# ningw42/GPU_Stereo_Matching

Measured on AMD Instinct MI355X. Metric: disparity-maps/sec + ms/frame, 1080p d_max=128, higher is better.
Workload: dtype u8; 1 GPU; cfg3: 1920x1080 synthetic rectified pairs, 11x11 SAD box aggregation + WTA (bit-exact with getDisp/kernalFindCorr), d_max=128; the path BASELINE.md's GPU-target table and the north star's >=100x CPU BlockMatching.cpp target are quoted on; BASELINE configs[2]'s guided-filter aggregation of the same frames: 'cfg3_guided'; width=1920, height=1080, num_disp=128, radius=5, seed=1234, parallelism=frame-parallel x1

## Files before the change

gpu_stereo_matching_amd/csrc/bm_box_mfma.hip:

```cpp
#include <atomic>
#include <type_traits>

#include "bm_common.h"

namespace sm {
namespace {

typedef _Float16 h2 __attribute__((ext_vector_type(2)));
typedef _Float16 h8 __attribute__((ext_vector_type(8)));
typedef float f4 __attribute__((ext_vector_type(4)));
typedef uint32_t u4 __attribute__((ext_vector_type(4)));

constexpr int kT = 64;
constexpr int kNW = 4;
constexpr int kThreads = 64 * kNW;
constexpr int kColB = 128;
constexpr uint32_t kInfBits = 0x7F800000u;

template <int R, int DMAX, int NP>
struct MG {
    static_assert(NP == 1 || NP == 2, "one or two disparities per pass");
    static constexpr int NOB = NP == 2 ? 3 : 4;
    static constexpr int NXB = (NP == 1 || R <= 6) ? 4 : 3;
    static constexpr int TOY = NOB == 4 ? kT - 2 * R : 16 * NOB;
    static constexpr int TOX = NXB == 4 ? kT - 2 * R : 16 * NXB;
    static constexpr int FOLD = 16 * NXB + 1;
    static constexpr int RC = kT + DMAX;
    static constexpr int RS_BYTES = RC * kColB;
    static constexpr int L_BYTES = kT * kColB;
    static constexpr int LDS_BYTES = L_BYTES + RS_BYTES;
    static constexpr int BIAS = ((2 * R + 1) * 255 + 1) / 2;
    static constexpr int KEEP = RC - TOX;
    static constexpr int NEW0 = KEEP & ~3;
    static constexpr int NEW4 = (RC - NEW0) / 4;
    static constexpr int MOVE_U = (KEEP * 8 + kThreads - 1) / kThreads;
    static_assert(TOY + 2 * R <= kT && TOX + 2 * R <= kT, "every output's window lies in the input tile");
    static_assert(8 * NEW4 + 8 * (kT / 4) <= kThreads, "a carried tile stages in one pass");
    static_assert(TOY * FOLD * 4 <= L_BYTES + TOX * kColB,
                  "the fold plane aliases the left tile and the band columns the next tile drops, none it keeps");
    static_assert(BIAS < 2048 && (2 * R + 1) * 255 - BIAS < 2048, "D1 exact in f16");
    static_assert((int64_t)(2 * R + 1) * (2 * R + 1) * 255 * 256 + 255 < (1 << 24), "keys exact in f32");
};

__device__ __forceinline__ int slot(int col, int q) { return col * kColB + ((q ^ ((col >> 1) & 7)) << 4); }

__device__ __forceinline__ uint32_t ld_u32(const uint8_t* p, int y, int x, int W, int H, int pitch) {
    if (y < 0 || y >= H) return 0u;
    const uint8_t* row = p + (int64_t)y * pitch;
    if (x >= 0 && x + 3 < W) {
        uint32_t v;
        __builtin_memcpy(&v, row + x, 4);
        return v;
    }
    uint32_t v = 0;
#pragma unroll
    for (int b = 0; b < 4; ++b)
        if (x + b >= 0 && x + b < W) v |= (uint32_t)row[x + b] << (8 * b);
    return v;
}

__device__ __forceinline__ void stage_pack(const uint32_t (&w)[8], uint8_t* dst, int col, int q) {
#pragma unroll
    for (int b = 0; b < 4; ++b) {
        u4 v;
#pragma unroll
        for (int m = 0; m < 4; ++m)
            v[m] = 0x64006400u | ((w[2 * m] >> (8 * b)) & 0xFFu) | (((w[2 * m + 1] >> (8 * b)) & 0xFFu) << 16);
        *reinterpret_cast<u4*>(dst + slot(col + b, q)) = v;
    }
}

template <int NC4>
__device__ __forceinline__ void stage_cols(const uint8_t* img, int ytop, int xleft, int W, int H, int pitch,
                                           uint8_t* dst, int tid) {
    for (int e = tid; e < 8 * NC4; e += kThreads) {
        const int q = e / NC4, j = e - q * NC4;
        uint32_t w[8];
#pragma unroll
        for (int i = 0; i < 8; ++i) w[i] = ld_u32(img, ytop + 8 * q + i, xleft + 4 * j, W, H, pitch);
        stage_pack(w, dst, 4 * j, q);
    }
}

template <int NEW0, int NEW4>
struct CarriedElem {
    bool right;
    int q, col, dx;
    __device__ __forceinline__ explicit CarriedElem(int tid) {
        constexpr int NR = 8 * NEW4, NL = 8 * (kT / 4);
        const int e = min(tid, NR + NL - 1);
        right = e < NR;
        const int el = e - NR;
        q = right ? e / NEW4 : el / (kT / 4);
        dx = 4 * (right ? e - q * NEW4 : el - q * (kT / 4));
        col = (right ? NEW0 : 0) + dx;
    }
};

__device__ __forceinline__ int per_tile(int tid) {
    asm volatile("" : "+v"(tid));
    return tid;
}

constexpr uint32_t kAbsBits = 0x7FFF7FFFu;

__device__ __forceinline__ u4 abs_diff(u4 l, u4 r, uint32_t keep) {
    u4 ad;
#pragma unroll
    for (int m = 0; m < 4; ++m) {
        const uint32_t lm = l[m], rm = r[m];
        const h2 d = __builtin_bit_cast(h2, lm) - __builtin_bit_cast(h2, rm);
        ad[m] = __builtin_bit_cast(uint32_t, d) & keep;
    }
    return ad;
}

__device__ __forceinline__ uint2 pack_f16(f4 v) {
    uint2 p;
    p.x = __builtin_bit_cast(uint32_t, __builtin_amdgcn_cvt_pkrtz(v[0], v[1]));
    p.y = __builtin_bit_cast(uint32_t, __builtin_amdgcn_cvt_pkrtz(v[2], v[3]));
    return p;
}

__device__ __forceinline__ f4 mfma(u4 a, u4 b, f4 c) {
    return __builtin_amdgcn_mfma_f32_16x16x32_f16(__builtin_bit_cast(h8, a), __builtin_bit_cast(h8, b), c, 0, 0, 0);
}

template <int R, int DMAX, int NP, bool WALK>
__device__ __forceinline__ void box_mfma_tiles(const MatchArgs& a, int tiles_x, int tiles_y, int per, int rem) {
    using G = MG<R, DMAX, NP>;
    constexpr int NXB = G::NXB, NOB = G::NOB;
    extern __shared__ __attribute__((aligned(16))) uint8_t smem[];
    uint8_t* lsm = smem;
    uint8_t* rsm = smem + G::L_BYTES;

    const int tid = threadIdx.x;
    const int wave = __builtin_amdgcn_readfirstlane(tid >> 6);
    const int lane = tid & 63;
    const int l16 = lane & 15;
    const int g = lane >> 4;

    const int wg = xcd_tile(blockIdx.x, gridDim.x);
    int t_begin = wg * per, t_end = t_begin + per;
    if (WALK && rem != 0) {
        t_begin += (int)((int64_t)wg * rem / (int)gridDim.x);
        t_end += (int)((int64_t)(wg + 1) * rem / (int)gridDim.x);
    }
    if constexpr (!WALK) t_end = t_begin + 1;
    if (t_begin >= t_end) return;
    const int tiles = tiles_x * tiles_y;
    int frame = t_begin / tiles;
    int ty = (t_begin - frame * tiles) / tiles_x;
    int tx = t_begin - frame * tiles - ty * tiles_x;
    const int W = a.W, H = a.H;
    const int d_lo = a.d_lo, d_hi = a.d_hi;

    u4 bv0, bvm, bvp;
    u4 bh, bhs;
#pragma unroll
    for (int m = 0; m < 4; ++m) {
        uint32_t w0 = 0, wm = 0, wp = 0, wh = 0, ws = 0;
#pragma unroll
        for (int e = 0; e < 2; ++e) {
            const int j = 2 * m + e;
            const int dv = 8 * g + j - l16;
            const int xin = j < 4 ? 4 * g + j : 16 + 4 * g + (j - 4);
            const int dh = xin - l16;
            const int ds = (j < 4 ? 16 + 4 * g + j : 4 * g + (j - 4)) - l16;
            w0 |= (dv >= 0 && dv <= 2 * R ? 0x3C00u : 0u) << (16 * e);
            wm |= (dv - 16 >= 0 && dv - 16 <= 2 * R ? 0x3C00u : 0u) << (16 * e);
            wp |= (dv + 16 >= 0 && dv + 16 <= 2 * R ? 0x3C00u : 0u) << (16 * e);
            wh |= (dh >= 0 && dh <= 2 * R ? 0x5C00u : 0u) << (16 * e);
            ws |= (ds >= 0 && ds <= 2 * R ? 0x5C00u : 0u) << (16 * e);
        }
        bv0[m] = w0;
        bvm[m] = wm;
        bvp[m] = wp;
        bh[m] = wh;
        bhs[m] = ws;
    }
    const float nbias = -(float)G::BIAS;
    const f4 c1 = {nbias, nbias, nbias, nbias};
    const float c2base = (float)(256 * (2 * R + 1) * G::BIAS);

    const int laddr = slot(l16, g);

    bool carried = false;
#pragma unroll 1
    for (int tile = t_begin;; ++tile) {
        const int x0 = tx * G::TOX;
        const int y0 = ty * G::TOY;
        const uint8_t* Lf = a.left + (int64_t)frame * a.frame_stride;
        const uint8_t* Rf = a.right + (int64_t)frame * a.frame_stride;

        if (!carried) {
            const int band0 = x0 - R - d_lo - DMAX;
            const int st = per_tile(tid);
            stage_cols<G::RC / 4>(Rf, y0 - R, band0, W, H, a.pitch, rsm, st);
            stage_cols<kT / 4>(Lf, y0 - R, x0 - R, W, H, a.pitch, lsm, st);
        }

        uint32_t best[NOB][NXB][4];
#pragma unroll
        for (int ob = 0; ob < NOB; ++ob)
#pragma unroll
            for (int xb = 0; xb < NXB; ++xb)
#pragma unroll
                for (int i = 0; i < 4; ++i) best[ob][xb][i] = kInfBits;

        const int d_end = min(d_hi, W - x0 + 1);
        const int nd = max(d_end - d_lo, 0);
        const int dw_lo = d_lo + (wave * nd) / kNW;
        const int dw_hi = d_lo + ((wave + 1) * nd) / kNW;
        const int d_free = W - (min(x0 + G::TOX, W) - 1);
        const int d_m = (x0 - R + kT > W) ? d_lo : max(min(x0 - R, d_free) + 1, d_lo);
        const int n_free = max(min(dw_hi, d_m) - dw_lo, 0);
        const int dw_m = dw_lo + n_free - n_free % NP;

        const bool carry_next = WALK && tile + 1 < t_end && tx + 1 < tiles_x;
        const int nxl = x0 + G::TOX - R, nxr = nxl - d_lo - DMAX + G::NEW0;
        const bool prefetch = carry_next && y0 - R >= 0 && y0 - R + kT <= H && nxr >= 0 && nxl + kT <= W;
        uint32_t pw[8];
        if (prefetch) {
            const CarriedElem<G::NEW0, G::NEW4> ce(per_tile(tid));
            const uint8_t* p = (ce.right ? Rf : Lf) + (int64_t)(y0 - R + 8 * ce.q) * a.pitch +
                               ((ce.right ? nxr : nxl) + ce.dx);
#pragma unroll
            for (int i = 0; i < 8; ++i) __builtin_memcpy(&pw[i], p + (int64_t)i * a.pitch, 4);
        }

        __syncthreads();

        auto run = [&](auto masked_c, const int lo, const int hi) {
            constexpr bool MASKED = decltype(masked_c)::value;
#pragma unroll 1
            for (int d = lo; d < hi; d += NP) {
                const int dd[2] = {d, min(d + 1, hi - 1)};
                int raddr[NP];
                float c2v[NP];
                f4 c2[NP];
#pragma unroll
                for (int p = 0; p < NP; ++p) {
                    raddr[p] = slot(l16 + DMAX + d_lo - dd[p], g);
                    c2v[p] = c2base + (float)dd[p];
                    c2[p] = f4{c2v[p], c2v[p], c2v[p], c2v[p]};
                }
                const int laddr_d = laddr + (int)((uint32_t)d >> 31);
                u4 t[NP][NOB];
#pragma unroll
                for (int cb = 0; cb <= NXB; ++cb) {
                    if (cb < 4) {
                        const u4 l0 = *reinterpret_cast<const u4*>(lsm + laddr_d + cb * 16 * kColB);
                        const u4 l1 = *reinterpret_cast<const u4*>(lsm + (laddr_d ^ 64) + cb * 16 * kColB);
#pragma unroll
                        for (int p = 0; p < NP; ++p) {
                            const u4 r0 = *reinterpret_cast<const u4*>(rsm + raddr[p] + cb * 16 * kColB);
                            const u4 r1 = *reinterpret_cast<const u4*>(rsm + (raddr[p] ^ 64) + cb * 16 * kColB);
                            uint32_t keep = kAbsBits;
                            if constexpr (MASKED) {
                                const int c0 = __builtin_amdgcn_readfirstlane(x0 - R + 16 * cb - dd[p]);
                                keep = (uint32_t)(l16 + c0) < (uint32_t)(W - dd[p]) ? kAbsBits : 0u;
                            }
                            const u4 ad0 = abs_diff(l0, r0, keep);
                            const u4 ad1 = abs_diff(l1, r1, keep);
                            f4 sv[4];
                            sv[0] = mfma(ad0, bv0, c1);
                            sv[1] = mfma(ad0, bvm, c1);
                            sv[1] = mfma(ad1, bvp, sv[1]);
                            sv[2] = mfma(ad1, bv0, c1);
                            if constexpr (NOB == 4) sv[3] = mfma(ad1, bvm, c1);
#pragma unroll
                            for (int ob = 0; ob < NOB; ++ob) {
                                const uint2 pk = pack_f16(sv[ob]);
                                t[p][ob][2 * (cb & 1)] = pk.x;
                                t[p][ob][2 * (cb & 1) + 1] = pk.y;
                            }
                        }
                    }
                    if constexpr (NP == 2) __builtin_amdgcn_sched_barrier(0);
                    if (cb >= 1) {
                        const int xb = cb - 1;
                        f4 c2x[NP];
#pragma unroll
                        for (int p = 0; p < NP; ++p) {
                            c2x[p] = c2[p];
                            if constexpr (MASKED) {
                                const int e = __builtin_amdgcn_readfirstlane(W - x0 - 16 * xb - dd[p]) - 4 * g;
#pragma unroll
                                for (int i = 0; i < 4; ++i)
                                    c2x[p][i] = i <= e ? c2v[p] : __builtin_bit_cast(float, kInfBits);
                            }
                        }
#pragma unroll
                        for (int ob = 0; ob < NOB; ++ob) {
                            u4 o[NP];
#pragma unroll
                            for (int p = 0; p < NP; ++p)
                                o[p] = __builtin_bit_cast(u4, mfma((cb & 1) ? bh : bhs, t[p][ob], c2x[p]));
#pragma unroll
                            for (int i = 0; i < 4; ++i) {
                                uint32_t k = o[0][i];
#pragma unroll
                                for (int p = 1; p < NP; ++p) k = min(k, o[p][i]);
                                best[ob][xb][i] = min(best[ob][xb][i], k);
                            }
                        }
                    }
                    if constexpr (NP == 2) __builtin_amdgcn_sched_barrier(0);
                }
            }
        };
        run(std::false_type{}, dw_lo, dw_m);
        run(std::true_type{}, dw_m, dw_hi);

        __syncthreads();

        uint32_t* fold = reinterpret_cast<uint32_t*>(smem);
        if (wave == 0) {
#pragma unroll
            for (int ob = 0; ob < NOB; ++ob)
#pragma unroll
                for (int xb = 0; xb < NXB; ++xb)
#pragma unroll
                    for (int i = 0; i < 4; ++i)
                        fold[(16 * ob + l16) * G::FOLD + 16 * xb + 4 * g + i] = best[ob][xb][i];
        }
        __syncthreads();
        if (wave != 0) {
#pragma unroll
            for (int ob = 0; ob < NOB; ++ob)
#pragma unroll
                for (int xb = 0; xb < NXB; ++xb)
#pragma unroll
                    for (int i = 0; i < 4; ++i)
                        atomicMin(&fold[(16 * ob + l16) * G::FOLD + 16 * xb + 4 * g + i], best[ob][xb][i]);
        }
        __syncthreads();
        uint8_t* Df = a.disp ? a.disp + (int64_t)frame * a.out_frame_stride : nullptr;
        uint32_t* Kf = a.keys ? a.keys + (int64_t)frame * W * H : nullptr;
        if (lane < G::TOX && x0 + lane < W) {
            const int ylim = min(G::TOY, H - y0);
            uint8_t* drow = Df ? Df + (int64_t)y0 * a.out_pitch + x0 + lane : nullptr;
            uint32_t* krow = Kf ? Kf + (int64_t)y0 * W + x0 + lane : nullptr;
            for (int j = wave; j < ylim; j += kNW) {
                const uint32_t kb = fold[j * G::FOLD + lane];
                const uint32_t kf = kb >= kInfBits ? 0xFFFFFFFFu : (uint32_t)__builtin_bit_cast(float, kb);
                const uint32_t k = min(kf, a.seed_key);
                if (drow) drow[(int64_t)j * a.out_pitch] = k < a.thresh_key ? (uint8_t)(k & 0xFFu) : (uint8_t)0;
                if (krow) krow[(int64_t)j * W] = k;
            }
        }

        if (tile + 1 == t_end) break;
        carried = carry_next;
        if (++tx == tiles_x) {
            tx = 0;
            if (++ty == tiles_y) {
                ty = 0;
                ++frame;
            }
        }
        if (!carried) {
            __syncthreads();
            continue;
        }
        const int mt = per_tile(tid);
        u4 mv[G::MOVE_U];
#pragma unroll
        for (int i = 0; i < G::MOVE_U; ++i) {
            const int u = min(mt + i * kThreads, G::KEEP * 8 - 1);
            mv[i] = *reinterpret_cast<const u4*>(rsm + slot((u >> 3) + G::TOX, u & 7));
        }
        __syncthreads();
#pragma unroll
        for (int i = 0; i < G::MOVE_U; ++i) {
            const int u = min(mt + i * kThreads, G::KEEP * 8 - 1);
            *reinterpret_cast<u4*>(rsm + slot(u >> 3, u & 7)) = mv[i];
        }
        const CarriedElem<G::NEW0, G::NEW4> ce(mt);
        if (!prefetch) {
#pragma unroll
            for (int i = 0; i < 8; ++i)
                pw[i] = ld_u32(ce.right ? Rf : Lf, y0 - R + 8 * ce.q + i, (ce.right ? nxr : nxl) + ce.dx, W, H,
                               a.pitch);
        }
        stage_pack(pw, ce.right ? rsm : lsm, ce.col, ce.q);
    }
}

template <int R, int DMAX, int NP>
__global__ __launch_bounds__(kThreads, 3) void box_mfma_kernel(MatchArgs a, int tiles_x, int tiles_y, int per,
                                                                int rem) {
    box_mfma_tiles<R, DMAX, NP, true>(a, tiles_x, tiles_y, per, rem);
}

template <int R, int DMAX>
__global__ __launch_bounds__(kThreads, 3) void box_mfma_tile_kernel(MatchArgs a, int tiles_x, int tiles_y) {
    box_mfma_tiles<R, DMAX, 1, false>(a, tiles_x, tiles_y, 1, 0);
}

constexpr int kMaxDevices = 64;
constexpr int kRangesPerSlot = 16;

template <int R, int DMAX, int NP>
hipError_t resident_workgroups(int* out) {
    static std::atomic<int> slots[kMaxDevices];
    int dev = 0;
    hipError_t e = hipGetDevice(&dev);
    if (e != hipSuccess) return e;
    const bool cached = dev >= 0 && dev < kMaxDevices;
    int v = cached ? slots[dev].load(std::memory_order_relaxed) : 0;
    if (v == 0) {
        int per_cu = 0, cus = 0;
        e = hipOccupancyMaxActiveBlocksPerMultiprocessor(&per_cu, box_mfma_kernel<R, DMAX, NP>, kThreads,
                                                         (size_t)MG<R, DMAX, NP>::LDS_BYTES);
        if (e != hipSuccess) return e;
        e = hipDeviceGetAttribute(&cus, hipDeviceAttributeMultiprocessorCount, dev);
        if (e != hipSuccess) return e;
        v = (per_cu > 0 ? per_cu : 1) * (cus > 0 ? cus : 1);
        if (cached) slots[dev].store(v, std::memory_order_relaxed);
    }
    *out = v;
    return hipSuccess;
}

template <int R, int DMAX, int NP>
hipError_t launch_rdp(const MatchArgs& a, int batch, hipStream_t s, int workgroups) {
    using G = MG<R, DMAX, NP>;
    const int tiles_x = (a.W + G::TOX - 1) / G::TOX;
    const int tiles_y = (a.H + G::TOY - 1) / G::TOY;
    const int64_t total = (int64_t)tiles_x * tiles_y * batch;
    if (total <= 0 || total > 0x7FFFFFFF || workgroups < 0) return hipErrorInvalidValue;
    int64_t n = workgroups;
    if constexpr (NP == 1) {
        if (n == 0 || n >= total) {
            hipLaunchKernelGGL((box_mfma_tile_kernel<R, DMAX>), dim3((unsigned)total), dim3(kThreads),
                               (size_t)G::LDS_BYTES, s, a, tiles_x, tiles_y);
            return hipGetLastError();
        }
    }
    if (n == 0) {
        int slots = 0;
        hipError_t e = resident_workgroups<R, DMAX, NP>(&slots);
        if (e != hipSuccess) return e;
        n = (int64_t)slots * kRangesPerSlot;
    }
    if (n > total) n = total;
    hipLaunchKernelGGL((box_mfma_kernel<R, DMAX, NP>), dim3((unsigned)n), dim3(kThreads), (size_t)G::LDS_BYTES, s, a,
                       tiles_x, tiles_y, (int)(total / n), (int)(total % n));
    return hipGetLastError();
}

template <int R, int DMAX>
hipError_t launch_rd(const MatchArgs& a, int batch, hipStream_t s, int workgroups) {
    if constexpr (DMAX == 64 && R <= 2) {
        if (a.d_hi - a.d_lo <= 32) return launch_rdp<R, DMAX, 1>(a, batch, s, workgroups);
    }
    return launch_rdp<R, DMAX, 2>(a, batch, s, workgroups);
}

template <int R>
hipError_t launch_r(const MatchArgs& a, int batch, hipStream_t s, int workgroups) {
    const int dspan = a.d_hi - a.d_lo;
    if (dspan <= 64) return launch_rd<R, 64>(a, batch, s, workgroups);
    if (dspan <= 128) return launch_rd<R, 128>(a, batch, s, workgroups);
    if (dspan <= 192) return launch_rd<R, 192>(a, batch, s, workgroups);
    return launch_rd<R, 256>(a, batch, s, workgroups);
}

}

bool box_mfma_scope(const MatchArgs& a) {
    return a.radius >= 1 && a.radius <= kMaxFastRadius && a.valid_mode == 0 && a.d_lo >= 0 && a.d_hi > a.d_lo &&
           a.d_hi <= kMaxDisp;
}

hipError_t launch_box_match_mfma(const MatchArgs& a, int batch, hipStream_t s, int workgroups) {
    if (!box_mfma_scope(a)) return hipErrorInvalidValue;
    switch (a.radius) {
        case 1: return launch_r<1>(a, batch, s, workgroups);
        case 2: return launch_r<2>(a, batch, s, workgroups);
        case 3: return launch_r<3>(a, batch, s, workgroups);
        case 4: return launch_r<4>(a, batch, s, workgroups);
        case 5: return launch_r<5>(a, batch, s, workgroups);
        case 6: return launch_r<6>(a, batch, s, workgroups);
        case 7: return launch_r<7>(a, batch, s, workgroups);
        default: return hipErrorInvalidValue;
    }
}

}
```

Before: 25990 disparity-maps/s.

## Hand-schedule paired-disparity MFMA loop and defer next-tile prefetch

Adds a dedicated unmasked loop for the two-disparities-per-pass path. It interleaves LDS fetches, f16 abs-diff, vertical and horizontal MFMA stages and min-reductions, with explicit sched_barrier slots so the next column block's loads and second-stage MFMAs overlap the first-stage work. For NP==2 the next-tile global prefetch is moved after the main loop instead of before it, which frees registers during the hot loop. The hand scheduling is rigid and may raise register pressure or serialise badly if the compiler's choices were already good.

```diff
diff --git a/gpu_stereo_matching_amd/csrc/bm_box_mfma.hip b/gpu_stereo_matching_amd/csrc/bm_box_mfma.hip
--- a/gpu_stereo_matching_amd/csrc/bm_box_mfma.hip
+++ b/gpu_stereo_matching_amd/csrc/bm_box_mfma.hip
@@ -221,13 +221,16 @@
         const int nxl = x0 + G::TOX - R, nxr = nxl - d_lo - DMAX + G::NEW0;
         const bool prefetch = carry_next && y0 - R >= 0 && y0 - R + kT <= H && nxr >= 0 && nxl + kT <= W;
         uint32_t pw[8];
-        if (prefetch) {
-            const CarriedElem<G::NEW0, G::NEW4> ce(per_tile(tid));
-            const uint8_t* p = (ce.right ? Rf : Lf) + (int64_t)(y0 - R + 8 * ce.q) * a.pitch +
-                               ((ce.right ? nxr : nxl) + ce.dx);
-#pragma unroll
-            for (int i = 0; i < 8; ++i) __builtin_memcpy(&pw[i], p + (int64_t)i * a.pitch, 4);
-        }
+        auto issue_prefetch = [&] {
+            if (prefetch) {
+                const CarriedElem<G::NEW0, G::NEW4> ce(per_tile(tid));
+                const uint8_t* p = (ce.right ? Rf : Lf) + (int64_t)(y0 - R + 8 * ce.q) * a.pitch +
+                                   ((ce.right ? nxr : nxl) + ce.dx);
+#pragma unroll
+                for (int i = 0; i < 8; ++i) __builtin_memcpy(&pw[i], p + (int64_t)i * a.pitch, 4);
+            }
+        };
+        if constexpr (NP == 1) issue_prefetch();
 
         __syncthreads();
 
@@ -310,7 +313,154 @@
                 }
             }
         };
-        run(std::false_type{}, dw_lo, dw_m);
+        auto run_paired = [&](auto np_c, const int lo, const int hi) {
+            static_assert(decltype(np_c)::value == 2 && NOB == 3, "the paired loop");
+            auto slot_end = [] { __builtin_amdgcn_sched_barrier(0); };
+            auto mins = [&](int ob, int x, const u4& o0, const u4& o1) {
+#pragma unroll
+                for (int i = 0; i < 4; ++i) best[ob][x][i] = min(best[ob][x][i], min(o0[i], o1[i]));
+            };
+#pragma unroll 1
+            for (int d = lo; d < hi; d += 2) {
+                const int dd[2] = {d, min(d + 1, hi - 1)};
+                int raddr[2];
+                f4 c2[2];
+#pragma unroll
+                for (int p = 0; p < 2; ++p) {
+                    raddr[p] = slot(l16 + DMAX + d_lo - dd[p], g);
+                    const float c2v = c2base + (float)dd[p];
+                    c2[p] = f4{c2v, c2v, c2v, c2v};
+                }
+                const int laddr_d = laddr + (int)((uint32_t)d >> 31);
+                u4 t[2][NOB];
+                u4 lq[2], rq[2][2];
+                auto fetch_l = [&](int cb, int c) {
+                    lq[c] = *reinterpret_cast<const u4*>(lsm + (laddr_d ^ (64 * c)) + cb * 16 * kColB);
+                };
+                auto fetch_r = [&](int cb, int p, int c) {
+                    rq[p][c] = *reinterpret_cast<const u4*>(rsm + (raddr[p] ^ (64 * c)) + cb * 16 * kColB);
+                };
+                auto fetch = [&](int cb, int c) {
+                    fetch_l(cb, c);
+                    fetch_r(cb, 0, c);
+                    fetch_r(cb, 1, c);
+                };
+                fetch(0, 0);
+                u4 om[2];
+#pragma unroll
+                for (int cb = 0; cb <= NXB; ++cb) {
+                    const bool s1 = cb < 4, s2 = cb >= 1;
+                    const int xb = cb - 1;
+                    u4 ad[2][2];
+                    f4 sv[2][NOB];
+                    u4 o[2][NOB];
+                    auto half = [&](int p, int c, int h) {
+#pragma unroll
+                        for (int m = 2 * h; m < 2 * h + 2; ++m) {
+                            const uint32_t lm = lq[c][m], rm = rq[p][c][m];
+                            const h2 df = __builtin_bit_cast(h2, lm) - __builtin_bit_cast(h2, rm);
+                            ad[p][c][m] = __builtin_bit_cast(uint32_t, df) & kAbsBits;
+                        }
+                    };
+                    auto cvt = [&](int p, int ob) {
+                        const uint2 pk = pack_f16(sv[p][ob]);
+                        t[p][ob][2 * (cb & 1)] = pk.x;
+                        t[p][ob][2 * (cb & 1) + 1] = pk.y;
+                    };
+                    auto stage2 = [&](int ob, int p) {
+                        o[p][ob] = __builtin_bit_cast(u4, mfma((cb & 1) ? bh : bhs, t[p][ob], c2[p]));
+                    };
+                    if (s1) {
+                        fetch_l(cb, 1);
+                        fetch_r(cb, 0, 1);
+                        half(0, 0, 0);
+                        half(0, 0, 1);
+                        if (cb >= 2) mins(1, xb - 1, om[0], om[1]);
+                        slot_end();
+                        fetch_r(cb, 1, 1);
+                        sv[0][0] = mfma(ad[0][0], bv0, c1);
+                        half(1, 0, 0);
+                        slot_end();
+                        sv[0][1] = mfma(ad[0][0], bvm, c1);
+                        half(1, 0, 1);
+                        slot_end();
+                        half(0, 1, 0);
+                        slot_end();
+                        sv[1][0] = mfma(ad[1][0], bv0, c1);
+                        half(0, 1, 1);
+                        slot_end();
+                        sv[1][1] = mfma(ad[1][0], bvm, c1);
+                        half(1, 1, 0);
+                        slot_end();
+                        sv[0][2] = mfma(ad[0][1], bv0, c1);
+                        half(1, 1, 1);
+                        slot_end();
+                        sv[0][1] = mfma(ad[0][1], bvp, sv[0][1]);
+                        cvt(0, 0);
+                        slot_end();
+                        sv[1][2] = mfma(ad[1][1], bv0, c1);
+                        cvt(1, 0);
+                        slot_end();
+                        sv[1][1] = mfma(ad[1][1], bvp, sv[1][1]);
+                        cvt(0, 2);
+                        slot_end();
+                        if (s2) stage2(0, 0);
+                        cvt(0, 1);
+                        slot_end();
+                        if (s2) stage2(0, 1);
+                        cvt(1, 2);
+                        slot_end();
+                        if (s2) stage2(2, 0);
+                        cvt(1, 1);
+                        slot_end();
+                        if (cb + 1 < 4) fetch(cb + 1, 0);
+                        if (s2) {
+                            stage2(1, 0);
+                            slot_end();
+                            stage2(2, 1);
+                            mins(0, xb, o[0][0], o[1][0]);
+                            slot_end();
+                            stage2(1, 1);
+                            slot_end();
+                            mins(2, xb, o[0][2], o[1][2]);
+                            slot_end();
+                            om[0] = o[0][1];
+                            om[1] = o[1][1];
+                        }
+                    } else {
+                        stage2(0, 0);
+                        stage2(0, 1);
+                        slot_end();
+                        stage2(2, 0);
+                        mins(1, xb - 1, om[0], om[1]);
+                        slot_end();
+                        stage2(2, 1);
+                        slot_end();
+                        stage2(1, 0);
+                        mins(0, xb, o[0][0], o[1][0]);
+                        slot_end();
+                        stage2(1, 1);
+                        slot_end();
+                        mins(2, xb, o[0][2], o[1][2]);
+                        slot_end();
+                        om[0] = o[0][1];
+                        om[1] = o[1][1];
+                    }
+                }
+                mins(1, NXB - 1, om[0], om[1]);
+                slot_end();
+            }
+        };
+        if constexpr (NP == 2) {
+            run_paired(std::integral_constant<int, NP>{}, dw_lo, dw_m);
+            if (!prefetch) {
+#pragma unroll
+                for (int i = 0; i < 8; ++i) pw[i] = 0;
+            }
+            issue_prefetch();
+        } else {
+            run(std::false_type{}, dw_lo, dw_m);
+        }
         run(std::true_type{}, dw_m, dw_hi);
 
         __syncthreads();
```

After: 26420 disparity-maps/s, median of 6. 1.02x the previous value.
